# OpenGene/AfterQC

Measured on AMD Instinct MI355X. Metric: Mreads/s (paired 2x150 bp) end-to-end good/bad split, higher is better.
Workload: dtype u8

## Files before the change

afterqc_amd/csrc/aqc_capi.hip:

```cpp
#include <hip/hip_runtime.h>

#include <cstdarg>
#include <cstdio>
#include <cstdlib>
#include <cstring>
#include <algorithm>
#include <atomic>
#include <mutex>
#include <vector>

#include "aqc_dev.hpp"
#include "aqc_kernels.hpp"
#include "aqc_fast.hpp"
#include "aqc_text.hpp"
#include "aqc_census.hpp"
#include "aqc_gzdev.hpp"
#include "aqc_gz.hpp"
#include <zlib.h>
#include <sys/mman.h>
#include <sched.h>
#include <pthread.h>
#include <cctype>

using namespace aqc;
// ... 74 lines not shown
    hipError_t e = hipStreamSynchronize(s.stream);
    const uint64_t g = s.qc.gen.load(std::memory_order_acquire);
    if (e == hipSuccess && s.qc.synced.load(std::memory_order_acquire) < g) {
        e = hipEventSynchronize(s.ev_qc);
        if (e == hipSuccess) {
            uint64_t seen = s.qc.synced.load(std::memory_order_relaxed);
            while (seen < g && !s.qc.synced.compare_exchange_weak(seen, g, std::memory_order_release)) { }
        }
    }
    return e;
}

constexpr uint64_t KMER_CAP = 1ull << 21;
constexpr uint64_t DENSE_CAP = (uint64_t)N_XCD * DENSE_ENTRIES;

struct QcDev {
    unsigned long long* acc = nullptr;
    KmerTable kt{};
    unsigned long long last_end = 0, epoch = 0;
};

}

struct __attribute__((visibility("hidden"))) aqc_ctx {
    bool force_generic = false;
    bool fuse_opt = false;
    bool qc_inline = false;
    int device = 0;
    int n_slots = 0;
    std::vector<Slot> slots;
    aqc_config cfg{};
    bool has_cfg = false;
    DevBuf circ[5];
    DevBuf kmer_partial;
    DevBuf gz_crc;
    hipStream_t qc_stream = nullptr;
    std::mutex qc_mu;
    DevCircles circles{};
    unsigned long long *counters = nullptr, *ovl_hist = nullptr, *dist_hist = nullptr;
    QcDev qc[4];
    int n_cu = 256;
    char name[256] = "";
};

struct StatusWords { int status; int pad_; unsigned long long err_key; };
static const StatusWords STATUS_CLEAR{0, 0, ~0ull};
static unsigned long long* err_key_of(const Slot& sl) { return reinterpret_cast<unsigned long long*>(sl.status + 2); }

static const char* status_text(int st, bool at_record) {
    if (st == AQC_ERR_ALPHABET) return "a base outside the reference's COMP table reached the correction walk (KeyError upstream)";
    if (at_record) {
        if (st == AQC_ERR_INDEX) return "the overlap walk read a quality line beyond its length — the line is shorter than its sequence line (IndexError upstream)";
        if (st == AQC_ERR_ARG) return "a name field the bubble filter converts with int() is not a number (ValueError upstream)";
    } else {
        if (st == AQC_ERR_READ_TOO_LONG) return "a read (or its quality line) is longer than AQC_MAX_READ_LEN";
        if (st == AQC_ERR_ARG) return "a read shorter than 5 bases reached statRead (IndexError upstream)";
        if (st == AQC_ERR_UNSUPPORTED) return "device limit exceeded (k-mer table full or string longer than 64)";
    }
    return "device-side error";
}

static int check_status(Slot& sl) {
    StatusWords w{0, 0, ~0ull};
    HIP_TRY(hipMemcpyAsync(&w, sl.status, sizeof(w), hipMemcpyDeviceToHost, sl.stream));
    HIP_TRY(hipStreamSynchronize(sl.stream));
    int st = w.status;
    if (st != 0) {
// ... 491 lines not shown
    else q.kt = t;
    return rc;
}

int aqc_qc_stat(aqc_ctx* c, int slot, int which, int mate, uint64_t first, uint64_t count, int post) {
    GET_SLOT(s);
    int rc;
    if (which < 0 || which > 3 || mate < 0 || mate > 1) return fail(AQC_ERR_ARG, "aqc_qc_stat: bad which/mate");
    if (!c->has_cfg) return fail(AQC_ERR_STATE, "aqc_qc_stat before aqc_set_config");
    if (first + count > s->n) return fail(AQC_ERR_ARG, "aqc_qc_stat: range exceeds the slot's %llu records", (unsigned long long)s->n);
    if (mate == 1 && !s->paired) return fail(AQC_ERR_ARG, "aqc_qc_stat: mate 1 of a single-end slot");
    if (post && !s->ran) return fail(AQC_ERR_STATE, "aqc_qc_stat(post) before aqc_run");
    if (count == 0) return 0;
    std::lock_guard<std::mutex> qc_lock(c->qc_mu);
    QcDev& q = c->qc[which];
    if ((rc = ensure_kmer(q))) return rc;
    hipStream_t qs = c->qc_inline ? s->stream : c->qc_stream;
    HIP_TRY(hipEventRecord(s->ev_main, s->stream));
    if (!c->qc_inline) HIP_TRY(hipStreamWaitEvent(qs, s->ev_main, 0));
    HIP_TRY(hipEventRecord(launch_event(*s, AQC_K_QC_STAT, 0), qs));
    const uint32_t mx = s->raw_max_len ? s->raw_max_len : AQC_MAX_READ_LEN;
    int cols = (int)((mx + 63) / 64 * 64);
    if (cols > AQC_QC_COLS) cols = AQC_QC_COLS;
    const size_t lds = sizeof(unsigned int) * (size_t)(QC_LDS_ROWS + 1) * cols + 16;
    uint64_t blocks = (count + QC_WPB - 1) / QC_WPB;
    if (blocks > (uint64_t)c->n_cu * 2) blocks = (uint64_t)c->n_cu * 2;
    const uint64_t need = (count + (QC_MAX_READS_PER_BLOCK - QC_WPB) - 1) / (QC_MAX_READS_PER_BLOCK - QC_WPB);
    if (blocks < need) blocks = need;
    const unsigned long long g0 = s->view.first_index + first;
    if (g0 < q.last_end) q.epoch++;
    q.last_end = g0 + count;
    const unsigned long long order_base = (q.epoch << 34) | g0;
    const uint32_t per_read = mx > (uint32_t)c->cfg.qc_kmer ? mx - (uint32_t)c->cfg.qc_kmer : 1;
    uint32_t rpr_max = 65535u / per_read;
    if (rpr_max < 1) rpr_max = 1;
    const uint64_t max_rounds = 512;
    const uint64_t rounds_per_block = (max_rounds + c->n_cu - 1) / c->n_cu;
    const bool fused = cols <= KMER_FUSED_MAX_COLS && rounds_per_block * rpr_max <= (uint64_t)QC_MAX_READS_PER_BLOCK;
    if (!fused || s->has_irregular)
        hipLaunchKernelGGL(qc_stat_kernel, dim3((unsigned)blocks), dim3(QC_BLOCK), lds, qs, s->view, mate, first, count, post,
                           (const aqc_result*)s->results.p, c->cfg.qc_kmer, q.acc, s->status, cols, fused ? 1 : 0);
    {
        uint64_t done = 0;
        while (done < count) {
            uint64_t chunk = count - done;
            if (chunk > max_rounds * rpr_max) chunk = max_rounds * rpr_max;
            uint64_t n_rounds64 = (chunk + rpr_max - 1) / rpr_max;
            if (n_rounds64 > (uint64_t)c->n_cu) {
                n_rounds64 = (n_rounds64 + c->n_cu - 1) / c->n_cu * c->n_cu;
                if (n_rounds64 > max_rounds) n_rounds64 = max_rounds;
            }
            const uint32_t rpr = (uint32_t)((chunk + n_rounds64 - 1) / n_rounds64);
            const uint32_t n_rounds = (uint32_t)((chunk + rpr - 1) / rpr);
            if (c->kmer_partial.reserve((size_t)n_rounds * DENSE_ENTRIES * sizeof(uint16_t))) return fail(AQC_ERR_HIP, "hipMalloc failed");
            unsigned kb = n_rounds < (unsigned)c->n_cu ? n_rounds : (unsigned)c->n_cu;
            hipLaunchKernelGGL(kmer_count_kernel, dim3(kb), dim3(KMER_BLOCK), fused ? KMER_FUSED_LDS_BYTES : KMER_LDS_BYTES, qs, s->view,
                               mate, first + done, chunk, post, (const aqc_result*)s->results.p, c->cfg.qc_kmer, q.kt, order_base + done,
                               (uint16_t*)c->kmer_partial.p, rpr, n_rounds, s->status, fused ? q.acc : (unsigned long long*)nullptr,
                               fused ? cols : 0);
            hipLaunchKernelGGL(kmer_reduce_kernel, dim3(DENSE_ENTRIES / KRED_ENTRIES), dim3(KRED_BLOCK), 0, qs,
                               (const uint16_t*)c->kmer_partial.p, n_rounds, q.kt, c->cfg.qc_kmer);
            done += chunk;
        }
    }
    HIP_TRY(hipGetLastError());
    HIP_TRY(hipEventRecord(launch_event(*s, AQC_K_QC_STAT, 1), qs));
    HIP_TRY(hipEventRecord(s->ev_qc, qs));
    s->qc.gen.fetch_add(1, std::memory_order_release);
    s->timed[AQC_K_QC_STAT] = !s->collecting;
    return 0;
}

struct FrameExtents { const aqc_text_extent* ext[2]; uint64_t n[2]; uint8_t last[2]; };
static int frame_impl(aqc_ctx* c, int slot, const aqc_text_chunk* ch, aqc_frame_info* info, bool resident, const FrameExtents* fx = nullptr) {
    GET_SLOT(s);
    if (!ch || !info || !ch->text1) return fail(AQC_ERR_ARG, "aqc_frame: null argument");
    const bool paired = ch->text2 != nullptr;
    const int nf = paired ? 2 : 1;
    const uint8_t* text[2] = {ch->text1, ch->text2};
    const uint64_t bytes[2] = {ch->bytes1, paired ? ch->bytes2 : 0};
    const int final_[2] = {ch->final1, ch->final2};
    for (int k = 0; k < nf; k++)
        if (bytes[k] >= (1ull << 31) - IDX_TILE) return fail(AQC_ERR_ARG, "aqc_frame: chunks must be < 2 GiB");
    HIP_TRY(slot_sync(*s));
    s->framed = s->formatted = false;
    s->ran = false;
    s->fused = false;
    DevBuf* arena[2] = {&s->seq1, &s->seq2};
    DevBuf* seq_off[2] = {&s->off1, &s->off2};
    DevBuf* qual_off[2] = {&s->qoff1, &s->qoff2};
    DevBuf* seq_len[2] = {&s->len1, &s->len2};
    if (s->t_scratch.reserve(256)) return fail(AQC_ERR_HIP, "hipMalloc failed");
    FrameMeta* d_meta = (FrameMeta*)s->t_scratch.p;
    unsigned long long* d_tot = (unsigned long long*)((uint8_t*)s->t_scratch.p + 64);
    uint64_t tiles[2] = {0, 0}, cap[2] = {0, 0};
    uint8_t* tbase[2] = {nullptr, nullptr};
    for (int k = 0; k < nf; k++) {
        const size_t slack = IDX_TILE + 64;
        if (arena[k]->reserve(TEXT_FRONT + bytes[k] + slack)) return fail(AQC_ERR_HIP, "hipMalloc of %llu bytes failed", (unsigned long long)bytes[k]);
        tbase[k] = (uint8_t*)arena[k]->p + TEXT_FRONT;
        if (!resident && fx && fx->n[k]) {
            uint64_t cur = 0;
            for (uint64_t e = 0; e < fx->n[k]; ++e) {
                const aqc_text_extent& x = fx->ext[k][e];
                if (x.offset < cur || x.offset + x.bytes > bytes[k] || !x.device_text) return fail(AQC_ERR_ARG, "aqc_frame_mixed: extents must be sorted, disjoint and inside the chunk");
                if (x.offset > cur) HIP_TRY(hipMemcpyAsync(tbase[k] + cur, text[k] + cur, x.offset - cur, hipMemcpyHostToDevice, s->stream));
                if (x.bytes) HIP_TRY(hipMemcpyAsync(tbase[k] + x.offset, x.device_text, x.bytes, hipMemcpyDeviceToDevice, s->stream));
                cur = x.offset + x.bytes;
            }
            if (bytes[k] > cur) HIP_TRY(hipMemcpyAsync(tbase[k] + cur, text[k] + cur, bytes[k] - cur, hipMemcpyHostToDevice, s->stream));
            HIP_TRY(hipMemsetAsync(tbase[k] + bytes[k], 0, slack, s->stream));
            s->last_byte[k] = bytes[k] ? fx->last[k] : (uint8_t)'\n';
        } else if (!resident) {
            if (bytes[k]) HIP_TRY(hipMemcpyAsync(tbase[k], text[k], bytes[k], hipMemcpyHostToDevice, s->stream));
            HIP_TRY(hipMemsetAsync(tbase[k] + bytes[k], 0, slack, s->stream));
            s->last_byte[k] = bytes[k] ? text[k][bytes[k] - 1] : (uint8_t)'\n';
        }
        tiles[k] = bytes[k] ? (bytes[k] + IDX_TILE - 1) / IDX_TILE : 1;
        const uint64_t guess = bytes[k] / 16 + 4096;
        cap[k] = s->t_line_end[k].cap / sizeof(uint32_t) > guess + 2 ? s->t_line_end[k].cap / sizeof(uint32_t) - 2 : guess;
        if (s->t_line_end[k].reserve(sizeof(uint32_t) * (cap[k] + 2))) return fail(AQC_ERR_HIP, "hipMalloc failed");
    }
    const uint64_t all_tiles = tiles[0] + (paired ? tiles[1] : 0);
    if (s->t_tile[0].reserve(sizeof(unsigned long long) * (all_tiles + 1))) return fail(AQC_ERR_HIP, "hipMalloc failed");
    const FrameMeta init{0xffffffffu, 0u, 0xffffffffu, 0u};
// ... 147 lines not shown
    const DevBuf* qo[2] = {&s->qoff1, &s->qoff2};
    for (int k = 0; k < (s->paired ? 2 : 1); k++) {
        v.f[k].text = (const uint8_t*)arena[k]->p + TEXT_FRONT;
        v.f[k].seq_off = (const uint32_t*)so[k]->p;
        v.f[k].qual_off = (const uint32_t*)qo[k]->p;
        v.f[k].seq_len = (const uint32_t*)sl[k]->p;
        v.f[k].name_off = (const uint32_t*)s->t_name_off[k].p;
        v.f[k].name_len = (const uint32_t*)s->t_name_len[k].p;
        v.f[k].plus_off = (const uint32_t*)s->t_plus_off[k].p;
        v.f[k].plus_len = (const uint32_t*)s->t_plus_len[k].p;
        v.f[k].qual_len = (const uint32_t*)s->t_qual_len[k].p;
        v.f[k].qview = (const uint32_t*)s->qview[k].p;
    }
    const uint64_t n_tiles = n ? (n + FMT_TILE - 1) / FMT_TILE : 1;
    const uint64_t n_super = (n_tiles + FMT_SUPER - 1) / FMT_SUPER;
    bool live[6];
    for (int q = 0; q < 6; q++) live[q] = (q < 3 || s->paired) && (q % 3 != 2 || v.store_overlap);
    unsigned long long h_tot[FMT_STREAMS] = {0, 0, 0, 0, 0, 0, 0, 0};
    if (s->fused && !plain && !spans && !v.store_overlap && n == s->n && n > 0) {
        unsigned long long misc[5];
        HIP_TRY(hipMemcpyAsync(misc, s->fz_misc.p, sizeof(misc), hipMemcpyDeviceToHost, s->stream));
        HIP_TRY(hipStreamSynchronize(s->stream));
        if ((misc[0] >> 32) == 0) {
            v.fused = 1;
            v.fstate[0] = (const uint32_t*)s->fz_rec[0].p; v.fstate[1] = (const uint32_t*)s->fz_rec[1].p;
            v.fbatch = (const unsigned long long*)s->fz_state.p;
            v.fbatch_shift = 5;
            static_assert(FastWaveLds<10, true, true>::PPW == 32, "fbatch_shift");
            h_tot[0] = misc[1]; h_tot[3] = misc[2]; h_tot[1] = misc[3]; h_tot[4] = misc[4];
        }
    }
    if (!v.fused) {
        s->fused = false;
        if (s->f_tile.reserve(sizeof(unsigned long long) * FMT_STREAMS * (n_tiles + n_super)) || s->t_scratch.reserve(256))
            return fail(AQC_ERR_HIP, "hipMalloc failed");
        unsigned long long* d_tot = (unsigned long long*)((uint8_t*)s->t_scratch.p + 128);
        unsigned long long* d_super = (unsigned long long*)s->f_tile.p + FMT_STREAMS * n_tiles;
        if (n) hipLaunchKernelGGL(fmt_tile_sums_kernel, dim3((unsigned)n_super), dim3(TXT_BLOCK), 0, s->stream, v, n, n_tiles, n_super, (unsigned long long*)s->f_tile.p, d_super);
        else HIP_TRY(hipMemsetAsync(s->f_tile.p, 0, sizeof(unsigned long long) * FMT_STREAMS * (n_tiles + n_super), s->stream));
        hipLaunchKernelGGL(fmt_tile_bases_kernel, dim3(v.spans ? FMT_STREAMS : 6), dim3(TXT_BLOCK), 0, s->stream, d_super, n_super, d_tot);
        HIP_TRY(hipGetLastError());
        HIP_TRY(hipMemcpyAsync(h_tot, d_tot, sizeof(unsigned long long) * (v.spans ? FMT_STREAMS : 6), hipMemcpyDeviceToHost, s->stream));
        HIP_TRY(hipStreamSynchronize(s->stream));
    }
    if (v.spans) {
        for (int f = 0; f < (s->paired ? 2 : 1); ++f) {
            s->n_events[f] = h_tot[FMT_EVENT_STREAM + f];
            if (s->f_events[f].reserve(sizeof(SpanEvent) * (s->n_events[f] + 1))) return fail(AQC_ERR_HIP, "hipMalloc failed");
        }
    }
    FormatOut outs{};
    for (int q = 0; q < 6; q++) {
        s->f_bytes[q] = live[q] ? h_tot[q] : 0;
        bytes_out[q] = s->f_bytes[q];
        if (s->f_out[q].reserve(s->f_bytes[q] + 64)) return fail(AQC_ERR_HIP, "hipMalloc failed");
        outs.p[q] = (uint8_t*)s->f_out[q].p;
    }
    if (n) {
        const uint64_t n_tasks = n * (s->paired ? 2 : 1);
        const uint64_t gen_cap = ((n_tiles + GEN_LISTS - 1) / GEN_LISTS) * FMT_TILE * (s->paired ? 2 : 1);
        const uint64_t plan0_bytes = (16 * n_tasks + 255) / 256 * 256;
        if (s->f_plan.reserve(plan0_bytes + 16 * PLAN_Q * gen_cap * GEN_LISTS) || s->f_patch.reserve(16 * n_tasks + 32 * gen_cap * GEN_LISTS) || s->f_over.reserve(sizeof(FmtTask) * n_tasks) ||
            s->f_pos.reserve(4 * gen_cap * GEN_LISTS + 2 * sizeof(unsigned int) * GEN_LISTS + 64))
            return fail(AQC_ERR_HIP, "hipMalloc failed");
        uint4* d_wplan = (uint4*)((uint8_t*)s->f_patch.p + 16 * n_tasks);
        unsigned int* d_ngen = (unsigned int*)((uint8_t*)s->f_pos.p + 4 * gen_cap * GEN_LISTS);
        unsigned int* d_nwhole = d_ngen + GEN_LISTS;
        const bool sparse = v.spans || v.fused;
        unsigned copy_blocks = (unsigned)((n_tasks + (COPY_BLOCK / 32) * FMT_UNROLL - 1) / ((COPY_BLOCK / 32) * FMT_UNROLL));
#ifdef AQC_COPY_PERSIST
        if (copy_blocks > (unsigned)c->n_cu * AQC_COPY_PERSIST) copy_blocks = (unsigned)c->n_cu * AQC_COPY_PERSIST;
#endif
        for (int pass = 0; pass < (v.store_overlap ? 2 : 1); ++pass) {
// ... 600 lines not shown
```

afterqc_amd/csrc/aqc_kernels.hpp:

```cpp
#pragma once
#include <hip/hip_runtime.h>
#include <stdint.h>

#include "../../include/afterqc_hip.h"

namespace aqc {

#ifdef AQC_FLAT_AS
#define AQC_GLOBAL_AS
#else
#define AQC_GLOBAL_AS __attribute__((address_space(1)))
#endif
typedef uint32_t aqc_u32x4_u __attribute__((ext_vector_type(4), aligned(1)));
typedef uint32_t aqc_u32x2_u __attribute__((ext_vector_type(2), aligned(1)));
typedef uint32_t aqc_u32_u __attribute__((aligned(1)));
typedef uint16_t aqc_u16_u __attribute__((aligned(1)));
__device__ __forceinline__ uint4 gload_u128(const uint8_t* p) {
    const aqc_u32x4_u t = *(const AQC_GLOBAL_AS aqc_u32x4_u*)p;
    return make_uint4(t.x, t.y, t.z, t.w);
}
__device__ __forceinline__ uint32_t gload_u32(const uint8_t* p) { return *(const AQC_GLOBAL_AS aqc_u32_u*)p; }
__device__ __forceinline__ void gstore_u128(uint8_t* p, uint4 v) {
    aqc_u32x4_u t;
    t.x = v.x; t.y = v.y; t.z = v.z; t.w = v.w;
// ... 987 lines not shown
        if (tn) {
            atomicAdd(&qc[AQC_QC_TOTAL_NUM * AQC_QC_COLS + i], tn);
            atomicAdd(&qc[AQC_QC_TOTAL_QUAL * AQC_QC_COLS + i], tq);
        }
        const unsigned int dv = accs[5 * cols + ci];
        if (dv) atomicAdd(&qc[AQC_QC_DISCONTINUITY * AQC_QC_COLS + i], (unsigned long long)dv);
        if (gch[i]) atomicAdd(&qc[AQC_QC_GC_HIST * AQC_QC_COLS + i], (unsigned long long)gch[i]);
    }
    if (threadIdx.x < 2 && scal[threadIdx.x]) atomicAdd(&qc[AQC_QC_SCALARS * AQC_QC_COLS + threadIdx.x], scal[threadIdx.x]);
}

#ifdef AQC_PROFILE
__device__ unsigned long long g_kprof[16];
#define KPROF_DECL unsigned long long kp_t[8] = {0, 0, 0, 0, 0, 0, 0, 0}; unsigned long long kp_last = __builtin_amdgcn_s_memtime();
#define KPROF(k) do { const unsigned long long now_ = __builtin_amdgcn_s_memtime(); kp_t[k] += now_ - kp_last; kp_last = now_; } while (0)
#define KPROF_FLUSH do { if (lane == 0) for (int k_ = 0; k_ < 8; ++k_) atomicAdd(&g_kprof[k_], kp_t[k_]); } while (0)
#else
#define KPROF_DECL
#define KPROF(k)
#define KPROF_FLUSH
#endif

constexpr int KMER_BLOCK = 1024;
constexpr int KMER_WPB = KMER_BLOCK / WAVE;
constexpr int KMER_EXQ = 1536;
constexpr size_t KMER_LDS_BYTES = DENSE_ENTRIES * 2 + (size_t)KMER_EXQ * 16 + 16;
constexpr int KMER_FUSED_MAX_COLS = 256;
constexpr size_t KMER_FUSED_LDS_BYTES = KMER_LDS_BYTES + sizeof(unsigned int) * (QC_LDS_ROWS + 1) * KMER_FUSED_MAX_COLS + 16;
constexpr int KMER_PASS_LANES = WAVE - 2;

__global__ __launch_bounds__(KMER_BLOCK) void kmer_count_kernel(DevBatch b, int mate, uint64_t first, uint64_t count, int post,
                                                                const aqc_result* __restrict__ results, int kmer_len,
                                                                KmerTable kt, unsigned long long order_base,
                                                                uint16_t* __restrict__ partial, uint32_t reads_per_round,
                                                                uint32_t n_rounds, int* status,
                                                                unsigned long long* __restrict__ qc ,
                                                                int cols) {
    extern __shared__ __attribute__((aligned(16))) unsigned int ktab[];
    unsigned long long* const exq_key = reinterpret_cast<unsigned long long*>(ktab + DENSE_ENTRIES / 2);
    unsigned long long* const exq_t = exq_key + KMER_EXQ;
    unsigned int* const exq_n = reinterpret_cast<unsigned int*>(exq_t + KMER_EXQ);
    const bool fused = qc != nullptr;
    unsigned int* const q_accs = exq_n + 4;
    unsigned int* const q_gch = q_accs + QC_LDS_ROWS * cols;
    unsigned long long* const q_scal = reinterpret_cast<unsigned long long*>(q_gch + cols);
    const QcLds qlds{q_accs, q_gch, q_scal, cols};
    const int lane = lane_id();
    const int wave = threadIdx.x / WAVE;
    if (fused) {
        for (int i = threadIdx.x; i < (QC_LDS_ROWS + 1) * cols; i += KMER_BLOCK) q_accs[i] = 0;
        if (threadIdx.x < 2) q_scal[threadIdx.x] = 0;
    }
    const unsigned long long kmask = kmer_len >= 8 ? ~0ull : (1ull << (8 * kmer_len)) - 1ull;
    auto exotic_insert = [&](unsigned long long key, unsigned long long t) {
        unsigned long long rkey = 0;
        for (int qq = 0; qq < kmer_len; qq++)
            rkey |= (unsigned long long)comp_or_n((uint8_t)(key >> (8 * (kmer_len - 1 - qq)))) << (8 * qq);
        long long h, hr;
        kmer_slot2(kt, key, rkey, h, hr);
        if (h < 0 || hr < 0) atomicCAS(status, 0, AQC_ERR_UNSUPPORTED);
        else {
            const unsigned long long oa = kt.order[h], ob = kt.order[hr];
            atomicAdd(&kt.counts[h], 1ull);
            if (oa > 2 * t) atomicMin(&kt.order[h], 2 * t);
            if (ob > 2 * t + 1) atomicMin(&kt.order[hr], 2 * t + 1);
        }
    };
    const uint32_t imask = (1u << (2 * kmer_len)) - 1u, kbits = (1u << kmer_len) - 1u;
    unsigned long long* const my_first = kt.dense_first + (size_t)xcc_id() * DENSE_ENTRIES;
    auto usable = [&](const ReadDesc& d) { return d.len >= 5 && d.len <= AQC_MAX_READ_LEN && d.len > kmer_len; };
    auto qc_usable = [&](const ReadDesc& d) { return fused && d.len >= 5 && d.len <= AQC_MAX_READ_LEN && d.len <= cols && d.qlen == d.len; };
    KPROF_DECL
    const bool complete = __syncthreads_and(threadIdx.x < (int)(DENSE_ENTRIES / KRED_ENTRIES) ? (int)kt.complete[threadIdx.x] : 1) != 0;
    constexpr uint32_t PAD = 0x41414141u;
    for (uint32_t round = blockIdx.x; round < n_rounds; round += gridDim.x) {
        for (int i = threadIdx.x; i < (int)(DENSE_ENTRIES / 2); i += KMER_BLOCK) ktab[i] = 0;
        if (threadIdx.x == 0) *exq_n = 0;
        __syncthreads();
        KPROF(0);
        const uint64_t r_lo = (uint64_t)round * reads_per_round;
        const uint64_t r_hi = min(r_lo + reads_per_round, count);
        for (uint64_t kb = r_lo + wave; kb < r_hi; kb += (uint64_t)KMER_WPB * WAVE) {
            const uint64_t myk = kb + (uint64_t)lane * KMER_WPB;
#if defined(__HIP_DEVICE_COMPILE__)
            const DevBatch __attribute__((address_space(4)))* kb_args = (const DevBatch __attribute__((address_space(4)))*)__builtin_amdgcn_kernarg_segment_ptr();
            asm volatile("" : "+s"(kb_args));
            const DevBatch bb = *kb_args;
#else
            const DevBatch bb = b;
#endif
            const ReadDesc mine = lane_desc(bb, mate, first + myk, myk < r_hi, post, results);
            const int nr = (int)min((uint64_t)WAVE, (r_hi - kb + KMER_WPB - 1) / KMER_WPB);
            ReadDesc cur = bcast_desc(mine, 0);
            uint32_t pre = PAD, pre_q = 0;
            if (qc_usable(cur) || usable(cur)) {
                pre = load4(reinterpret_cast<const uint8_t*>(cur.s), 4 * lane, cur.len, PAD);
                if (fused) pre_q = load4(reinterpret_cast<const uint8_t*>(cur.q), 4 * lane, cur.qlen, 0);
            }
            KPROF(1);
            for (int r = 0; r < nr; ++r) {
                uint32_t ws = pre;
                const uint32_t wq0 = pre_q;
                ReadDesc nxt = cur;
                if (r + 1 < nr) {
                    nxt = bcast_desc(mine, r + 1);
                    if (qc_usable(nxt) || usable(nxt)) {
                        pre = load4(reinterpret_cast<const uint8_t*>(nxt.s), 4 * lane, nxt.len, PAD);
                        if (fused) pre_q = load4(reinterpret_cast<const uint8_t*>(nxt.q), 4 * lane, nxt.qlen, 0);
                    }
// ... 48 lines not shown
                            for (int j = 0; j < 4; ++j) {
                                const unsigned long long t = t0 + (unsigned long long)(x + j);
                                if (dense[j] && seen[j] > t) __hip_atomic_fetch_min(&my_first[idx[j]], t, __ATOMIC_RELAXED, __HIP_MEMORY_SCOPE_WORKGROUP);
                            }
                        }
                        KPROF(4);
                        if (__ballot(badwin != 0u)) {
                            const uint32_t w1 = (uint32_t)__shfl_down(ws, 1), w2 = (uint32_t)__shfl_down(ws, 2);
#pragma unroll
                            for (int j = 0; j < 4; ++j) {
                                if (exotic[j]) {
                                    const uint32_t lo = __builtin_amdgcn_alignbit(w1, ws, 8 * j), hi = __builtin_amdgcn_alignbit(w2, w1, 8 * j);
                                    const unsigned long long key = (((unsigned long long)hi << 32) | lo) & kmask;
                                    const unsigned long long t = t0 + (unsigned long long)(x + j);
                                    const unsigned int slot = atomicAdd(exq_n, 1u);
                                    if (slot < (unsigned int)KMER_EXQ) { exq_key[slot] = key; exq_t[slot] = t; }
                                    else exotic_insert(key, t);
                                }
                            }
                        }
                    }
                }
                KPROF(5);
                cur = nxt;
            }
        }
        __syncthreads();
        KPROF(6);
        {
            const unsigned int nq = min(*exq_n, (unsigned int)KMER_EXQ);
            for (unsigned int e = threadIdx.x; e < nq; e += KMER_BLOCK) exotic_insert(exq_key[e], exq_t[e]);
        }
        KPROF(5);
        uint4* dst = reinterpret_cast<uint4*>(partial + (size_t)round * DENSE_ENTRIES);
        const uint4* srcv = reinterpret_cast<const uint4*>(ktab);
        for (int i = threadIdx.x; i < (int)(DENSE_ENTRIES * 2 / 16); i += KMER_BLOCK) dst[i] = srcv[i];
        __builtin_amdgcn_s_waitcnt(0xc07f);
        __builtin_amdgcn_s_barrier();
        KPROF(7);
    }
    if (fused) {
        __syncthreads();
        const int cq = cols >> 2;
        for (int i = threadIdx.x; i < cols; i += KMER_BLOCK) {
            const int ci = (i & 3) * cq + (i >> 2);
            unsigned long long tn = 0, tq = 0;
#pragma unroll
            for (int row = 0; row < 5; ++row) {
                const unsigned int v = q_accs[row * cols + ci];
                const unsigned long long cnt = v >> 20, qs = (v & 0xfffffu) - 33ull * cnt;
                if (row < 4 && v) {
                    atomicAdd(&qc[(AQC_QC_BASE_COUNT_A + row) * AQC_QC_COLS + i], cnt);
                    atomicAdd(&qc[(AQC_QC_BASE_QUAL_A + row) * AQC_QC_COLS + i], qs);
                }
                tn += cnt; tq += qs;
            }
            if (tn) {
                atomicAdd(&qc[AQC_QC_TOTAL_NUM * AQC_QC_COLS + i], tn);
                atomicAdd(&qc[AQC_QC_TOTAL_QUAL * AQC_QC_COLS + i], tq);
            }
            const unsigned int dv = q_accs[5 * cols + ci];
            if (dv) atomicAdd(&qc[AQC_QC_DISCONTINUITY * AQC_QC_COLS + i], (unsigned long long)dv);
            if (q_gch[i]) atomicAdd(&qc[AQC_QC_GC_HIST * AQC_QC_COLS + i], (unsigned long long)q_gch[i]);
        }
        if (threadIdx.x < 2 && q_scal[threadIdx.x]) atomicAdd(&qc[AQC_QC_SCALARS * AQC_QC_COLS + threadIdx.x], q_scal[threadIdx.x]);
    }
    KPROF_FLUSH;
}

__global__ __launch_bounds__(KRED_BLOCK) void kmer_reduce_kernel(const uint16_t* __restrict__ partial, uint32_t n_rounds,
                                                                 KmerTable kt, int kmer_len) {
    __shared__ unsigned int part[4][KRED_ENTRIES];
    const int quad = threadIdx.x & 63, grp = threadIdx.x >> 6;
    const uint32_t e0 = blockIdx.x * KRED_ENTRIES + 4 * quad;
    unsigned int s0 = 0, s1 = 0, s2 = 0, s3 = 0;
#pragma unroll 8
    for (uint32_t r = grp; r < n_rounds; r += 4) {
        const uint2 v = *reinterpret_cast<const uint2*>(partial + (size_t)r * DENSE_ENTRIES + e0);
        s0 += v.x & 0xffffu; s1 += v.x >> 16; s2 += v.y & 0xffffu; s3 += v.y >> 16;
    }
    part[grp][4 * quad + 0] = s0; part[grp][4 * quad + 1] = s1; part[grp][4 * quad + 2] = s2; part[grp][4 * quad + 3] = s3;
    __syncthreads();
    const int i = threadIdx.x;
    const uint32_t idx = blockIdx.x * KRED_ENTRIES + i;
    kt.dense_count[idx] += part[0][i] + part[1][i] + part[2][i] + part[3][i];
    bool seen = idx >= (1u << (2 * kmer_len));
    if (!kt.complete[blockIdx.x]) {
        for (int x = 0; x < N_XCD && !seen; ++x) seen = kt.dense_first[(size_t)x * DENSE_ENTRIES + idx] != ~0ull;
        const int all = __syncthreads_and(seen ? 1 : 0);
        if (threadIdx.x == 0 && all) kt.complete[blockIdx.x] = 1u;
    }
}

__global__ void kmer_compact_kernel(KmerTable kt, unsigned long long* keys, unsigned long long* counts,
                                    unsigned long long* order, unsigned long long cap, unsigned long long* n_out) {
    const uint64_t i = (uint64_t)blockIdx.x * blockDim.x + threadIdx.x;
    if (i > kt.mask + 1) return;
    const unsigned long long key = i > kt.mask ? 0ull : kt.keys[i];
    if (i > kt.mask ? kt.order[i] == ~0ull : key == 0) return;
    const unsigned long long w = atomicAdd(n_out, 1ull);
    if (w < cap) { keys[w] = key; counts[w] = kt.counts[i]; order[w] = kt.order[i]; }
}

__global__ void kmer_compact_dense_kernel(KmerTable kt, int k, unsigned long long* keys, unsigned long long* counts,
                                          unsigned long long* order, unsigned long long cap, unsigned long long* n_out) {
    const uint32_t i = blockIdx.x * blockDim.x + threadIdx.x;
    if (i >= (1u << (2 * k))) return;
    const unsigned long long never = ~0ull;
    unsigned long long f = never, fr = never, cnt = 0;
    const uint32_t ir = dense_rc(i, k);
    for (int x = 0; x < N_XCD; ++x) {
        const unsigned long long a = kt.dense_first[(size_t)x * DENSE_ENTRIES + i], b = kt.dense_first[(size_t)x * DENSE_ENTRIES + ir];
        f = a < f ? a : f;
        fr = b < fr ? b : fr;
        cnt += kt.dense_count[(size_t)x * DENSE_ENTRIES + i];
    }
    if (f == never && fr == never) return;
    unsigned long long ord = never;
    if (f != never) ord = 2 * f;
    if (fr != never && 2 * fr + 1 < ord) ord = 2 * fr + 1;
    unsigned long long key = 0;
    for (int j = 0; j < k; ++j) {
        const uint32_t code = (i >> (2 * j)) & 3u;
        key |= (unsigned long long)((CODE_TO_BASE >> (8 * code)) & 0xffu) << (8 * j);
// ... 123 lines not shown
```

afterqc_amd/csrc/aqc_text.hpp:

```cpp
#pragma once
#include <hip/hip_runtime.h>
#include <stdint.h>

#include "afterqc_hip.h"
#include "aqc_kernels.hpp"
#include "aqc_fast.hpp"

namespace aqc {

constexpr int TXT_BLOCK = 256;
constexpr int TXT_BYTES_PER_THREAD = 64;
constexpr int TXT_TILE = TXT_BLOCK * TXT_BYTES_PER_THREAD;
constexpr int SCAN_ITEMS = 16;
constexpr int SCAN_TILE = TXT_BLOCK * SCAN_ITEMS;

__device__ __forceinline__ unsigned long long block_excl_scan(unsigned long long v, unsigned long long* lds ,
                                                              unsigned long long& total) {
    const int lane = lane_id(), wave = threadIdx.x / WAVE;
    unsigned long long inc = v;
#pragma unroll
    for (int d = 1; d < WAVE; d <<= 1) {
        const unsigned long long o = __shfl_up(inc, d);
        if (lane >= d) inc += o;
    }
// ... 579 lines not shown
        }
    }
    const uint32_t body = nlen + (plw & LEN_MASK) + 4u;
    uint32_t qlen = len;
    if (slw & LEN_IRR) {
        int qs_, ql_;
        irregular_quality_slice(t, r, v.plain, 0, 0, qs_, ql_);
        qlen = (uint32_t)ql_;
    }
    sz[0] = (flag == AQC_GOOD && !whole) ? body + len + qlen : 0u;
    sz[1] = flag == AQC_GOOD ? 0u : body + (uint32_t)FLAG_TEXT_LEN[flag] + len + qlen;
    sz[2] = 0u;
    if (v.store_overlap) {
        const uint4 w1 = *(reinterpret_cast<const uint4*>(v.results + r) + 1);
        if (in_overlap_stream(v, w0, w1)) {
            const uint32_t olen = v.plain ? len : (w0.w & 0xffffu);
            uint32_t oq = v.plain ? qlen : olen;
            if ((slw & LEN_IRR) && !v.plain) {
                int qs_, ql_;
                irregular_quality_slice(t, r, 0, 1, (int)olen, qs_, ql_);
                oq = (uint32_t)ql_;
            }
            sz[2] = body + olen + oq;
        }
    }
}

constexpr int FMT_TILE = 128;
constexpr int FMT_SUPER = 8;
constexpr int FMT_STREAMS = 8;
constexpr int FMT_EVENT_STREAM = 6;

__global__ __launch_bounds__(TXT_BLOCK) void fmt_tile_sums_kernel(FormatView v, uint64_t n, uint64_t n_tiles, uint64_t n_super,
                                                                  unsigned long long* __restrict__ tile_sum, unsigned long long* __restrict__ super_sum) {
    constexpr int HALVES = FMT_SUPER * FMT_TILE / WAVE;
    constexpr int ROUNDS = FMT_SUPER * FMT_TILE / TXT_BLOCK;
    static_assert(FMT_TILE == 2 * WAVE && HALVES * WAVE == ROUNDS * TXT_BLOCK, "a tile is two waves' records");
    __shared__ uint32_t part[HALVES][FMT_STREAMS];
    const int lane = lane_id(), wave = threadIdx.x / WAVE;
    const int nfiles = v.paired ? 2 : 1;
    for (int i = threadIdx.x; i < HALVES * FMT_STREAMS; i += TXT_BLOCK) (&part[0][0])[i] = 0u;
    __syncthreads();
    const uint64_t r0 = (uint64_t)blockIdx.x * (FMT_SUPER * FMT_TILE);
#pragma unroll 1
    for (int it = 0; it < ROUNDS; ++it) {
        const uint64_t r = r0 + (uint64_t)it * TXT_BLOCK + threadIdx.x;
        const int half = it * (TXT_BLOCK / WAVE) + wave;
        if (r0 + (uint64_t)half * WAVE >= n) break;
        for (int file = 0; file < nfiles; ++file) {
            uint32_t sz[3] = {0, 0, 0}, ev = 0;
            if (r < n) fmt_sizes(v, r, file, sz, ev);
            const int g = wave_sum_u((int)sz[0]), b = wave_sum_u((int)sz[1]);
            if (lane == 0) { part[half][file * 3 + 0] = (uint32_t)g; part[half][file * 3 + 1] = (uint32_t)b; }
            if (v.store_overlap) {
                const int o = wave_sum_u((int)sz[2]);
                if (lane == 0) part[half][file * 3 + 2] = (uint32_t)o;
            }
            if (v.spans) {
                const int e = wave_sum_u((int)ev);
                if (lane == 0) part[half][FMT_EVENT_STREAM + file] = (uint32_t)e;
            }
        }
    }
    __syncthreads();
    if (threadIdx.x < FMT_STREAMS) {
        const int q = threadIdx.x;
        unsigned long long run = 0;
        for (int t = 0; t < FMT_SUPER; ++t) {
            const uint64_t tile = (uint64_t)blockIdx.x * FMT_SUPER + t;
            if (tile < n_tiles) tile_sum[(uint64_t)q * n_tiles + tile] = run;
            run += (unsigned long long)part[2 * t][q] + part[2 * t + 1][q];
        }
        super_sum[(uint64_t)q * n_super + blockIdx.x] = run;
    }
}

__global__ __launch_bounds__(TXT_BLOCK) void fmt_tile_bases_kernel(unsigned long long* __restrict__ tile_sum, uint64_t n_tiles,
                                                                   unsigned long long* __restrict__ total_out) {
    __shared__ unsigned long long lds[4];
    constexpr int PER = 8;
    unsigned long long* ts = tile_sum + (uint64_t)blockIdx.x * n_tiles;
    unsigned long long carry = 0;
    for (uint64_t t0 = 0; t0 < n_tiles; t0 += (uint64_t)TXT_BLOCK * PER) {
        const uint64_t t = t0 + (uint64_t)threadIdx.x * PER;
        unsigned long long val[PER], sum = 0;
#pragma unroll
        for (int k = 0; k < PER; ++k) {
            val[k] = t + k < n_tiles ? ts[t + k] : 0ull;
            sum += val[k];
        }
        unsigned long long total;
        unsigned long long run = carry + block_excl_scan(sum, lds, total);
#pragma unroll
        for (int k = 0; k < PER; ++k) {
            if (t + k < n_tiles) ts[t + k] = run;
            run += val[k];
        }
        carry += total;
    }
    if (threadIdx.x == 0) total_out[blockIdx.x] = carry;
}

__device__ __forceinline__ void store16u(uint8_t* p, uint4 v) { __builtin_memcpy(p, &v, 16); }
__device__ __forceinline__ uint4 load16u_t(const uint8_t* p) {
    uint4 v;
    __builtin_memcpy(&v, p, 16);
    return v;
}

constexpr int FMT_MAXP = 10;
#ifndef AQC_GEN_ALIGN
#define AQC_GEN_ALIGN 1
#endif
#ifndef AQC_GEN_SMALL
#define AQC_GEN_SMALL 1
#endif
#ifndef AQC_GEN_DECODE_LDS
#define AQC_GEN_DECODE_LDS 1
#endif
constexpr uint32_t GRID_MIN = 48;
__host__ __device__ constexpr uint32_t piece_items(uint32_t len) {
    return len >= 16u ? ((len + 15u) >> 4) + ((AQC_GEN_ALIGN && len >= GRID_MIN) ? 1u : 0u) : (len > 0u ? 1u : 0u);
}
constexpr uint32_t FMT_LIT_BIT = 0x80000000u;
struct FmtPiece {
    uint32_t src;
    uint16_t dst, len;
};
struct FmtTask {
    uint32_t pos;
    uint8_t stream;
    uint8_t np, n_patch, pad_;
    uint16_t total, items;
// ... 775 lines not shown
```

Before: 60.86.

## Fold k-mer partial reduction into count kernel and fuse tile-base scan via ticket

The k-mer count kernel no longer writes per-round 16-bit partial tables to global memory for a separate reduce kernel. It keeps one LDS table across rounds, spills counts near 16-bit overflow through atomics, and atomically adds the final counts into per-XCD global counters. A slimmer kernel now only updates the completeness flags. Separately, the format tile-sum kernel uses a last-block ticket to run the super-tile base scan itself, which removes the fmt_tile_bases launch. This trades partial-buffer traffic and launches for global atomics, halves reads per round with doubled max rounds, and adds a ticket word in scratch that must be zeroed and reset.

After: 60.33. About the same (-0.9%).

```diff
diff --git a/afterqc_amd/csrc/aqc_capi.hip b/afterqc_amd/csrc/aqc_capi.hip
--- a/afterqc_amd/csrc/aqc_capi.hip
+++ b/afterqc_amd/csrc/aqc_capi.hip
@@ -130,7 +130,6 @@
     aqc_config cfg{};
     bool has_cfg = false;
     DevBuf circ[5];
-    DevBuf kmer_partial;
     DevBuf gz_crc;
     hipStream_t qc_stream = nullptr;
     std::mutex qc_mu;
@@ -688,9 +687,9 @@
     q.last_end = g0 + count;
     const unsigned long long order_base = (q.epoch << 34) | g0;
     const uint32_t per_read = mx > (uint32_t)c->cfg.qc_kmer ? mx - (uint32_t)c->cfg.qc_kmer : 1;
-    uint32_t rpr_max = 65535u / per_read;
+    uint32_t rpr_max = 32767u / per_read;
     if (rpr_max < 1) rpr_max = 1;
-    const uint64_t max_rounds = 512;
+    const uint64_t max_rounds = 1024;
     const uint64_t rounds_per_block = (max_rounds + c->n_cu - 1) / c->n_cu;
     const bool fused = cols <= KMER_FUSED_MAX_COLS && rounds_per_block * rpr_max <= (uint64_t)QC_MAX_READS_PER_BLOCK;
     if (!fused || s->has_irregular)
@@ -708,14 +707,11 @@
             }
             const uint32_t rpr = (uint32_t)((chunk + n_rounds64 - 1) / n_rounds64);
             const uint32_t n_rounds = (uint32_t)((chunk + rpr - 1) / rpr);
-            if (c->kmer_partial.reserve((size_t)n_rounds * DENSE_ENTRIES * sizeof(uint16_t))) return fail(AQC_ERR_HIP, "hipMalloc failed");
             unsigned kb = n_rounds < (unsigned)c->n_cu ? n_rounds : (unsigned)c->n_cu;
             hipLaunchKernelGGL(kmer_count_kernel, dim3(kb), dim3(KMER_BLOCK), fused ? KMER_FUSED_LDS_BYTES : KMER_LDS_BYTES, qs, s->view,
                                mate, first + done, chunk, post, (const aqc_result*)s->results.p, c->cfg.qc_kmer, q.kt, order_base + done,
-                               (uint16_t*)c->kmer_partial.p, rpr, n_rounds, s->status, fused ? q.acc : (unsigned long long*)nullptr,
-                               fused ? cols : 0);
-            hipLaunchKernelGGL(kmer_reduce_kernel, dim3(DENSE_ENTRIES / KRED_ENTRIES), dim3(KRED_BLOCK), 0, qs,
-                               (const uint16_t*)c->kmer_partial.p, n_rounds, q.kt, c->cfg.qc_kmer);
+                               rpr, n_rounds, s->status, fused ? q.acc : (unsigned long long*)nullptr, fused ? cols : 0);
+            hipLaunchKernelGGL(kmer_complete_kernel, dim3(DENSE_ENTRIES / KRED_ENTRIES), dim3(KRED_BLOCK), 0, qs, q.kt, c->cfg.qc_kmer);
             done += chunk;
         }
     }
@@ -725,6 +721,14 @@
     s->qc.gen.fetch_add(1, std::memory_order_release);
     s->timed[AQC_K_QC_STAT] = !s->collecting;
     return 0;
+}
+
+constexpr size_t T_SCRATCH_TICKET = 240;
+static_assert(128 + sizeof(FrameOut) <= T_SCRATCH_TICKET && 128 + sizeof(unsigned long long) * FMT_STREAMS <= T_SCRATCH_TICKET, "the ticket has its own bytes");
+static int scratch_ready(Slot& s) {
+    if (s.t_scratch.p) return 0;
+    if (s.t_scratch.reserve(256)) return -1;
+    return hipMemsetAsync(s.t_scratch.p, 0, 256, s.stream) == hipSuccess ? 0 : -1;
 }
 
 struct FrameExtents { const aqc_text_extent* ext[2]; uint64_t n[2]; uint8_t last[2]; };
@@ -746,7 +750,7 @@
     DevBuf* seq_off[2] = {&s->off1, &s->off2};
     DevBuf* qual_off[2] = {&s->qoff1, &s->qoff2};
     DevBuf* seq_len[2] = {&s->len1, &s->len2};
-    if (s->t_scratch.reserve(256)) return fail(AQC_ERR_HIP, "hipMalloc failed");
+    if (scratch_ready(*s)) return fail(AQC_ERR_HIP, "hipMalloc failed");
     FrameMeta* d_meta = (FrameMeta*)s->t_scratch.p;
     unsigned long long* d_tot = (unsigned long long*)((uint8_t*)s->t_scratch.p + 64);
     uint64_t tiles[2] = {0, 0}, cap[2] = {0, 0};
@@ -960,13 +964,16 @@
     }
     if (!v.fused) {
         s->fused = false;
-        if (s->f_tile.reserve(sizeof(unsigned long long) * FMT_STREAMS * (n_tiles + n_super)) || s->t_scratch.reserve(256))
+        if (s->f_tile.reserve(sizeof(unsigned long long) * FMT_STREAMS * (n_tiles + n_super)) || scratch_ready(*s))
             return fail(AQC_ERR_HIP, "hipMalloc failed");
         unsigned long long* d_tot = (unsigned long long*)((uint8_t*)s->t_scratch.p + 128);
         unsigned long long* d_super = (unsigned long long*)s->f_tile.p + FMT_STREAMS * n_tiles;
-        if (n) hipLaunchKernelGGL(fmt_tile_sums_kernel, dim3((unsigned)n_super), dim3(TXT_BLOCK), 0, s->stream, v, n, n_tiles, n_super, (unsigned long long*)s->f_tile.p, d_super);
-        else HIP_TRY(hipMemsetAsync(s->f_tile.p, 0, sizeof(unsigned long long) * FMT_STREAMS * (n_tiles + n_super), s->stream));
-        hipLaunchKernelGGL(fmt_tile_bases_kernel, dim3(v.spans ? FMT_STREAMS : 6), dim3(TXT_BLOCK), 0, s->stream, d_super, n_super, d_tot);
+        if (n) hipLaunchKernelGGL(fmt_tile_sums_kernel, dim3((unsigned)n_super), dim3(TXT_BLOCK), 0, s->stream, v, n, n_tiles, n_super, (unsigned long long*)s->f_tile.p, d_super,
+                                  d_tot, (unsigned int*)((uint8_t*)s->t_scratch.p + T_SCRATCH_TICKET));
+        else {
+            HIP_TRY(hipMemsetAsync(s->f_tile.p, 0, sizeof(unsigned long long) * FMT_STREAMS * (n_tiles + n_super), s->stream));
+            HIP_TRY(hipMemsetAsync(d_tot, 0, sizeof(unsigned long long) * FMT_STREAMS, s->stream));
+        }
         HIP_TRY(hipGetLastError());
         HIP_TRY(hipMemcpyAsync(h_tot, d_tot, sizeof(unsigned long long) * (v.spans ? FMT_STREAMS : 6), hipMemcpyDeviceToHost, s->stream));
         HIP_TRY(hipStreamSynchronize(s->stream));
diff --git a/afterqc_amd/csrc/aqc_kernels.hpp b/afterqc_amd/csrc/aqc_kernels.hpp
--- a/afterqc_amd/csrc/aqc_kernels.hpp
+++ b/afterqc_amd/csrc/aqc_kernels.hpp
@@ -1043,8 +1043,7 @@
 __global__ __launch_bounds__(KMER_BLOCK) void kmer_count_kernel(DevBatch b, int mate, uint64_t first, uint64_t count, int post,
                                                                 const aqc_result* __restrict__ results, int kmer_len,
                                                                 KmerTable kt, unsigned long long order_base,
-                                                                uint16_t* __restrict__ partial, uint32_t reads_per_round,
-                                                                uint32_t n_rounds, int* status,
+                                                                uint32_t reads_per_round, uint32_t n_rounds, int* status,
                                                                 unsigned long long* __restrict__ qc ,
                                                                 int cols) {
     extern __shared__ __attribute__((aligned(16))) unsigned int ktab[];
@@ -1079,13 +1078,14 @@
     };
     const uint32_t imask = (1u << (2 * kmer_len)) - 1u, kbits = (1u << kmer_len) - 1u;
     unsigned long long* const my_first = kt.dense_first + (size_t)xcc_id() * DENSE_ENTRIES;
+    unsigned int* const my_count = kt.dense_count + (size_t)xcc_id() * DENSE_ENTRIES;
     auto usable = [&](const ReadDesc& d) { return d.len >= 5 && d.len <= AQC_MAX_READ_LEN && d.len > kmer_len; };
     auto qc_usable = [&](const ReadDesc& d) { return fused && d.len >= 5 && d.len <= AQC_MAX_READ_LEN && d.len <= cols && d.qlen == d.len; };
     KPROF_DECL
     const bool complete = __syncthreads_and(threadIdx.x < (int)(DENSE_ENTRIES / KRED_ENTRIES) ? (int)kt.complete[threadIdx.x] : 1) != 0;
     constexpr uint32_t PAD = 0x41414141u;
+    for (int i = threadIdx.x; i < (int)(DENSE_ENTRIES / 2); i += KMER_BLOCK) ktab[i] = 0;
     for (uint32_t round = blockIdx.x; round < n_rounds; round += gridDim.x) {
-        for (int i = threadIdx.x; i < (int)(DENSE_ENTRIES / 2); i += KMER_BLOCK) ktab[i] = 0;
         if (threadIdx.x == 0) *exq_n = 0;
         __syncthreads();
         KPROF(0);
@@ -1200,12 +1200,29 @@
             for (unsigned int e = threadIdx.x; e < nq; e += KMER_BLOCK) exotic_insert(exq_key[e], exq_t[e]);
         }
         KPROF(5);
-        uint4* dst = reinterpret_cast<uint4*>(partial + (size_t)round * DENSE_ENTRIES);
-        const uint4* srcv = reinterpret_cast<const uint4*>(ktab);
-        for (int i = threadIdx.x; i < (int)(DENSE_ENTRIES * 2 / 16); i += KMER_BLOCK) dst[i] = srcv[i];
+        uint4* const tabv = reinterpret_cast<uint4*>(ktab);
+        for (int i = threadIdx.x; i < (int)(DENSE_ENTRIES * 2 / 16); i += KMER_BLOCK) {
+            const uint4 w = tabv[i];
+            if ((w.x | w.y | w.z | w.w) & 0x80008000u) {
+                const uint32_t ww[4] = {w.x, w.y, w.z, w.w};
+#pragma unroll
+                for (int j = 0; j < 4; ++j) {
+                    if (ww[j] & 0x00008000u) atomicAdd(&my_count[8 * i + 2 * j], 0x8000u);
+                    if (ww[j] & 0x80000000u) atomicAdd(&my_count[8 * i + 2 * j + 1], 0x8000u);
+                }
+                tabv[i] = make_uint4(w.x & 0x7fff7fffu, w.y & 0x7fff7fffu, w.z & 0x7fff7fffu, w.w & 0x7fff7fffu);
+            }
+        }
         __builtin_amdgcn_s_waitcnt(0xc07f);
         __builtin_amdgcn_s_barrier();
         KPROF(7);
+    }
+    {
+        const uint16_t* const tab16 = reinterpret_cast<const uint16_t*>(ktab);
+        for (uint32_t e = threadIdx.x; e < DENSE_ENTRIES; e += KMER_BLOCK) {
+            const unsigned int cnt = tab16[e];
+            if (cnt) __hip_atomic_fetch_add(&my_count[e], cnt, __ATOMIC_RELAXED, __HIP_MEMORY_SCOPE_WORKGROUP);
+        }
     }
     if (fused) {
         __syncthreads();
@@ -1236,28 +1253,13 @@
     KPROF_FLUSH;
 }
 
-__global__ __launch_bounds__(KRED_BLOCK) void kmer_reduce_kernel(const uint16_t* __restrict__ partial, uint32_t n_rounds,
-                                                                 KmerTable kt, int kmer_len) {
-    __shared__ unsigned int part[4][KRED_ENTRIES];
-    const int quad = threadIdx.x & 63, grp = threadIdx.x >> 6;
-    const uint32_t e0 = blockIdx.x * KRED_ENTRIES + 4 * quad;
-    unsigned int s0 = 0, s1 = 0, s2 = 0, s3 = 0;
-#pragma unroll 8
-    for (uint32_t r = grp; r < n_rounds; r += 4) {
-        const uint2 v = *reinterpret_cast<const uint2*>(partial + (size_t)r * DENSE_ENTRIES + e0);
-        s0 += v.x & 0xffffu; s1 += v.x >> 16; s2 += v.y & 0xffffu; s3 += v.y >> 16;
-    }
-    part[grp][4 * quad + 0] = s0; part[grp][4 * quad + 1] = s1; part[grp][4 * quad + 2] = s2; part[grp][4 * quad + 3] = s3;
-    __syncthreads();
-    const int i = threadIdx.x;
-    const uint32_t idx = blockIdx.x * KRED_ENTRIES + i;
-    kt.dense_count[idx] += part[0][i] + part[1][i] + part[2][i] + part[3][i];
+__global__ __launch_bounds__(KRED_BLOCK) void kmer_complete_kernel(KmerTable kt, int kmer_len) {
+    if (kt.complete[blockIdx.x]) return;
+    const uint32_t idx = blockIdx.x * KRED_ENTRIES + threadIdx.x;
     bool seen = idx >= (1u << (2 * kmer_len));
-    if (!kt.complete[blockIdx.x]) {
-        for (int x = 0; x < N_XCD && !seen; ++x) seen = kt.dense_first[(size_t)x * DENSE_ENTRIES + idx] != ~0ull;
-        const int all = __syncthreads_and(seen ? 1 : 0);
-        if (threadIdx.x == 0 && all) kt.complete[blockIdx.x] = 1u;
-    }
+    for (int x = 0; x < N_XCD && !seen; ++x) seen = kt.dense_first[(size_t)x * DENSE_ENTRIES + idx] != ~0ull;
+    const int all = __syncthreads_and(seen ? 1 : 0);
+    if (threadIdx.x == 0 && all) kt.complete[blockIdx.x] = 1u;
 }
 
 __global__ void kmer_compact_kernel(KmerTable kt, unsigned long long* keys, unsigned long long* counts,
diff --git a/afterqc_amd/csrc/aqc_text.hpp b/afterqc_amd/csrc/aqc_text.hpp
--- a/afterqc_amd/csrc/aqc_text.hpp
+++ b/afterqc_amd/csrc/aqc_text.hpp
@@ -635,11 +635,14 @@
 constexpr int FMT_EVENT_STREAM = 6;
 
 __global__ __launch_bounds__(TXT_BLOCK) void fmt_tile_sums_kernel(FormatView v, uint64_t n, uint64_t n_tiles, uint64_t n_super,
-                                                                  unsigned long long* __restrict__ tile_sum, unsigned long long* __restrict__ super_sum) {
+                                                                  unsigned long long* __restrict__ tile_sum, unsigned long long* super_sum,
+                                                                  unsigned long long* __restrict__ total_out, unsigned int* ticket) {
     constexpr int HALVES = FMT_SUPER * FMT_TILE / WAVE;
     constexpr int ROUNDS = FMT_SUPER * FMT_TILE / TXT_BLOCK;
     static_assert(FMT_TILE == 2 * WAVE && HALVES * WAVE == ROUNDS * TXT_BLOCK, "a tile is two waves' records");
     __shared__ uint32_t part[HALVES][FMT_STREAMS];
+    __shared__ unsigned long long lds[4];
+    __shared__ unsigned int last;
     const int lane = lane_id(), wave = threadIdx.x / WAVE;
     const int nfiles = v.paired ? 2 : 1;
     for (int i = threadIdx.x; i < HALVES * FMT_STREAMS; i += TXT_BLOCK) (&part[0][0])[i] = 0u;
@@ -676,32 +679,48 @@
         }
         super_sum[(uint64_t)q * n_super + blockIdx.x] = run;
     }
-}
-
-__global__ __launch_bounds__(TXT_BLOCK) void fmt_tile_bases_kernel(unsigned long long* __restrict__ tile_sum, uint64_t n_tiles,
-                                                                   unsigned long long* __restrict__ total_out) {
-    __shared__ unsigned long long lds[4];
+    if (threadIdx.x == 0) last = 0u;
+    if (wave == 0) {
+        asm volatile("s_waitcnt vmcnt(0)" ::: "memory");
+        if (lane == 0) {
+            __threadfence();
+            asm volatile("s_waitcnt vmcnt(0)" ::: "memory");
+            const unsigned int drawn = __hip_atomic_fetch_add(ticket, 1u, __ATOMIC_RELAXED, __HIP_MEMORY_SCOPE_AGENT);
+            if (drawn == (unsigned int)gridDim.x - 1u) last = 1u;
+        }
+    }
+    __syncthreads();
+    if (!last) return;
+    __threadfence();
+    asm volatile("s_waitcnt vmcnt(0)" ::: "memory");
     constexpr int PER = 8;
-    unsigned long long* ts = tile_sum + (uint64_t)blockIdx.x * n_tiles;
-    unsigned long long carry = 0;
-    for (uint64_t t0 = 0; t0 < n_tiles; t0 += (uint64_t)TXT_BLOCK * PER) {
-        const uint64_t t = t0 + (uint64_t)threadIdx.x * PER;
-        unsigned long long val[PER], sum = 0;
-#pragma unroll
-        for (int k = 0; k < PER; ++k) {
-            val[k] = t + k < n_tiles ? ts[t + k] : 0ull;
-            sum += val[k];
-        }
-        unsigned long long total;
-        unsigned long long run = carry + block_excl_scan(sum, lds, total);
-#pragma unroll
-        for (int k = 0; k < PER; ++k) {
-            if (t + k < n_tiles) ts[t + k] = run;
-            run += val[k];
-        }
-        carry += total;
-    }
-    if (threadIdx.x == 0) total_out[blockIdx.x] = carry;
+#pragma unroll 1
+    for (int q = 0; q < FMT_STREAMS; ++q) {
+        const bool live = q >= FMT_EVENT_STREAM ? (v.spans && q - FMT_EVENT_STREAM < nfiles) : (q / 3 < nfiles && (q % 3 != 2 || v.store_overlap));
+        unsigned long long carry = 0;
+        if (live) {
+            unsigned long long* ts = super_sum + (uint64_t)q * n_super;
+            for (uint64_t t0 = 0; t0 < n_super; t0 += (uint64_t)TXT_BLOCK * PER) {
+                const uint64_t t = t0 + (uint64_t)threadIdx.x * PER;
+                unsigned long long val[PER], sum = 0;
+#pragma unroll
+                for (int k = 0; k < PER; ++k) {
+                    val[k] = t + k < n_super ? ts[t + k] : 0ull;
+                    sum += val[k];
+                }
+                unsigned long long total;
+                unsigned long long run = carry + block_excl_scan(sum, lds, total);
+#pragma unroll
+                for (int k = 0; k < PER; ++k) {
+                    if (t + k < n_super) ts[t + k] = run;
+                    run += val[k];
+                }
+                carry += total;
+            }
+        }
+        if (threadIdx.x == 0) total_out[q] = carry;
+    }
+    if (threadIdx.x == 0) __hip_atomic_store(ticket, 0u, __ATOMIC_RELAXED, __HIP_MEMORY_SCOPE_AGENT);
 }
 
 __device__ __forceinline__ void store16u(uint8_t* p, uint4 v) { __builtin_memcpy(p, &v, 16); }
```
